# zyc-123/InstanceDiff

Measured on AMD Instinct MI355X. Metric: denoising steps/sec (256x256 bs16), higher is better.
Workload: dtype f32; 1 GPU; 256x256 1-ch synthetic, 1000-step reverse chain, batch 16 per GPU, 2 UNet fwd + reverse update per step; global_batch=16, parallelism=replicas x1 (no collective)

## Files before the change

### instancediff_amd/csrc/conv_wino4.hip

```cpp
#include "conv_args.h"
#include "wino_common.h"

using idiff_detail::ConvArgs;

namespace {

using namespace idiff_wino;

constexpr int CK = 4;
constexpr int TW = 32, TH = 16;
constexpr int RCOLS = TW + 2;
constexpr int RS = 40;
constexpr int TRH = TH + 2;
constexpr int PS = TRH * RS;
constexpr int PSP = 768;
constexpr int NT = 512;
constexpr int NL = 6;
constexpr int R_FLOATS = NL * NT;
constexpr int V_FLOATS = 9 * 2 * 64 * 4;
constexpr int U_FLOATS = 9 * 4 * 64 * 4;

typedef float floatx2 __attribute__((ext_vector_type(2)));

struct Geo4 {
    int np;
    int total;
    int tiles_y8;
};

#ifdef IDIFF_WINO_SLOTS
#define SLOT_INIT long long sl_acc[10] = {0, 0, 0, 0, 0, 0, 0, 0, 0, 0}, sl_t = 0;
#define SLOT_START sl_t = __builtin_readcyclecounter();
#define SLOT_MARK(k)                                        \
    {                                                       \
        const long long t_ = __builtin_readcyclecounter();  \
        sl_acc[k] += t_ - sl_t;                             \
        sl_t = t_;                                          \
    }
#define SLOT_FINI                                                                                                                   \
    if (lane == 0) {                                                                                                                \
        long long w_ = 0;                                                                                                           \
        for (int q_ = 0; q_ < 9; ++q_) w_ += sl_acc[q_];                                                                            \
        atomicAdd((unsigned long long*)trace + 8 + 2 * wave, (unsigned long long)w_);                                               \
        atomicAdd((unsigned long long*)trace + 9 + 2 * wave, (unsigned long long)sl_acc[9]);                                        \
    }
#else
#define SLOT_INIT
#define SLOT_START
#define SLOT_MARK(k)
#define SLOT_FINI
#endif

template <int MODE, int SPEC, bool RAG, bool HEAVY, bool G16>
__device__ __forceinline__ void conv_wino4_body(const ConvArgs& a, const Geo4& g, float* smem TRACE_PARAM) {
    static_assert(!G16 || (MODE == IDIFF_CONV_NORMAL && SPEC != 2), "the 16-byte gather: contiguous pieces, LDS-DMA only");
    constexpr int HU = G16 ? 5 : 4, HR = 3;
    constexpr int N_U = HEAVY ? HU : 9 - HU;
    constexpr int NR = G16 ? (HEAVY ? HR : 3 - HR) : NL;
    float* const Rb = smem;
    float* const Vb = smem + 3 * R_FLOATS;
    float* const Ub = Vb + 2 * V_FLOATS;
    float* const econst = Ub + 2 * U_FLOATS;
    int* const gtab = reinterpret_cast<int*>(econst + 512);
    constexpr unsigned R_BYTES = R_FLOATS * 4, U_BYTES = U_FLOATS * 4;
    const unsigned lds_base = __builtin_amdgcn_readfirstlane((unsigned)reinterpret_cast<unsigned long long>(smem));
    const unsigned U_LDS0 = lds_base + (3 * R_FLOATS + 2 * V_FLOATS) * 4;

    const int tid = threadIdx.x;
    const int lane = tid & 63;
    const int wave = __builtin_amdgcn_readfirstlane(tid >> 6);
    const int k4 = lane >> 4;
    const int cb = wave & 3;
    const int tblk = wave >> 2;
    const int g16_u0 = HEAVY ? wave : 4 * HU + wave - 4, g16_r0 = HEAVY ? wave : 4 * HR + wave - 4;
    const int HWin = a.Hin * a.Win;
    const int nchunks = a.Cin / CK;

    constexpr int RSRC_FLAGS = 0x00020000;
    struct View {
        int b, co0, y0, x0;
    };
    const float *p0A = a.src0, *p1A = a.src0, *puA = a.wwino4, *p0B = a.src0, *p1B = a.src0, *puB = a.wwino4;
    View vA = {0, 0, 0, 0}, vB = {0, 0, 0, 0};
    int nrB = 0;
    unsigned omaskA = 0, omaskB = 0;
    int it_b = 0, it_cob = 0, it_px = 0, it_py = 0;
    const int tiles_y = g.np / a.tiles_x;
    int d_cob, d_px, d_py, d_b;
    {
        const int G0 = gridDim.x;
        d_cob = G0 % a.ncob;
        const int r1 = G0 / a.ncob;
        d_px = r1 % a.tiles_x;
        const int r2 = r1 / a.tiles_x;
        d_py = r2 % tiles_y;
        d_b = r2 / tiles_y;
    }
    auto decode_first = [&](int item) {
        it_cob = item % a.ncob;
        const int r1 = item / a.ncob;
        it_px = r1 % a.tiles_x;
        const int r2 = r1 / a.tiles_x;
        it_py = r2 % tiles_y;
        it_b = r2 / tiles_y;
    };
    auto advance_item = [&]() {
        it_cob += d_cob;
        int carry = it_cob >= a.ncob;
        it_cob -= carry ? a.ncob : 0;
        it_px += d_px + carry;
        carry = it_px >= a.tiles_x;
        it_px -= carry ? a.tiles_x : 0;
        it_py += d_py + carry;
        carry = it_py >= tiles_y;
        it_py -= carry ? tiles_y : 0;
        it_b += d_b + carry;
    };
    auto decode_B = [&]() {
        vB.b = it_b, vB.co0 = it_cob * 64, vB.y0 = it_py * TH, vB.x0 = it_px * TW;
        puB = scalar_ptr(a.wwino4 + (long long)it_cob * U_FLOATS);
        p0B = scalar_ptr(a.src0 + (long long)it_b * a.bs0);
        p1B = scalar_ptr(SPEC == 3 ? a.src1 + (long long)it_b * a.bs1 : a.src0);
        nrB = 0x7fffffff;
    };
    auto write_table = [&](const View& v) {
        unsigned om;
        if (G16) gather_decode16<NT, NR, 256, PSP / 4, PS / 4, RS / 4>(tid, g16_r0 * 64 + lane, om, v.y0, v.x0, a, gtab, HWin);
        else gather_decode<MODE, NT, NL, PSP, PS, RS, RCOLS>(tid, om, v.y0, v.x0, a, gtab, HWin);
        return om;
    };
    auto shift_B_to_A = [&]() { p0A = p0B, p1A = p1B, puA = puB, vA = vB, omaskA = omaskB; };
    const int ustride_b = a.ncob * U_FLOATS * 4;

    typedef const __attribute__((address_space(4))) floatx4* cfloatx4p;
    struct Pro {
        floatx4 a, b;
    };
    auto load_pro = [&](int p) {
        Pro r;
        if (SPEC == 2) {
            const bool inA = p < nchunks;
            const long long o = (long long)(inA ? vA.b : vB.b) * a.C0r + (inA ? p : p - nchunks) * CK;
            r.a = *(cfloatx4p)(a.pro_a + o);
            r.b = *(cfloatx4p)(a.pro_b + o);
        }
        return r;
    };

    const unsigned u_voff = tid * 16;
    const unsigned l_voff = lane * 16;
    auto dma_u_piece16 = [&](int p, int buf, int i) {
        const bool inA = p < nchunks;
        const unsigned ub = (unsigned)(g16_u0 + 4 * i) * 1024u;
        const int so = (inA ? p : p - nchunks) * ustride_b + (int)ub;
        const __amdgpu_buffer_rsrc_t rsu = __builtin_amdgcn_make_buffer_rsrc(const_cast<float*>(inA ? puA : puB), 0, inA ? 0x7fffffff : nrB, RSRC_FLAGS);
        const unsigned lds0 = __builtin_amdgcn_readfirstlane(U_LDS0 + (unsigned)buf * U_BYTES + ub);
        asm volatile("s_nop 4\n\ts_mov_b32 m0, %2\n\ts_nop 0\n\tbuffer_load_dwordx4 %0, %1, %3 offen lds" ::"v"(l_voff), "s"(rsu), "s"(lds0), "s"(so) : "memory");
    };
    auto dma_u = [&](int p, int buf) {
        if (G16) {
#pragma unroll
            for (int i = 0; i < N_U; ++i) dma_u_piece16(p, buf, i);
            return;
        }
        const bool inA = p < nchunks;
        const int so = (inA ? p : p - nchunks) * ustride_b;
        const __amdgpu_buffer_rsrc_t rsu = __builtin_amdgcn_make_buffer_rsrc(const_cast<float*>(inA ? puA : puB), 0, inA ? 0x7fffffff : nrB, RSRC_FLAGS);
        const unsigned lds0 = __builtin_amdgcn_readfirstlane(U_LDS0 + (unsigned)buf * U_BYTES + (unsigned)wave * 1024u);
        asm volatile(
            "s_nop 4\n\ts_mov_b32 m0, %2\n\ts_nop 0\n\tbuffer_load_dwordx4 %0, %1, %3 offen lds\n\t"
            "s_add_u32 m0, m0, 0x2000\n\ts_nop 0\n\tbuffer_load_dwordx4 %0, %1, %4 offen lds\n\t"
            "s_add_u32 m0, m0, 0x2000\n\ts_nop 0\n\tbuffer_load_dwordx4 %0, %1, %5 offen lds\n\t"
            "s_add_u32 m0, m0, 0x2000\n\ts_nop 0\n\tbuffer_load_dwordx4 %0, %1, %6 offen lds"
            ::"v"(u_voff), "s"(rsu), "s"(lds0), "s"(so), "s"(so + NT * 16), "s"(so + 2 * NT * 16), "s"(so + 3 * NT * 16)
            : "memory", "scc");
        if (!HEAVY) {
            const unsigned lds4 = __builtin_amdgcn_readfirstlane(lds0 + 4 * NT * 16 - 256 * 16);
            asm volatile("s_nop 4\n\ts_mov_b32 m0, %2\n\ts_nop 0\n\tbuffer_load_dwordx4 %0, %1, %3 offen lds" ::"v"(u_voff), "s"(rsu), "s"(lds4),
                         "s"(so + 4 * NT * 16 - 256 * 16)
                         : "memory");
        }
    };
    auto dma_u_piece = [&](int p, int buf, int i) {
        if (G16) return dma_u_piece16(p, buf, i);
        const bool inA = p < nchunks;
        const int so = (inA ? p : p - nchunks) * ustride_b + (i < 4 ? i * NT * 16 : 4 * NT * 16 - 256 * 16);
        const __amdgpu_buffer_rsrc_t rsu = __builtin_amdgcn_make_buffer_rsrc(const_cast<float*>(inA ? puA : puB), 0, inA ? 0x7fffffff : nrB, RSRC_FLAGS);
        const unsigned lds0 = __builtin_amdgcn_readfirstlane(U_LDS0 + (unsigned)buf * U_BYTES + (unsigned)wave * 1024u + (unsigned)(i < 4 ? i * NT * 16 : 4 * NT * 16 - 256 * 16));
        asm volatile("s_nop 4\n\ts_mov_b32 m0, %2\n\ts_nop 0\n\tbuffer_load_dwordx4 %0, %1, %3 offen lds" ::"v"(u_voff), "s"(rsu), "s"(lds0), "s"(so) : "memory");
    };
    auto dma_raw = [&](int p, unsigned rslot) {
        const bool inA = p < nchunks;
        const int cbase = (inA ? p : p - nchunks) * CK;
        int goff[NL];
#pragma unroll
        for (int i = 0; i < NL; ++i) goff[i] = gtab[i * NT + tid];
        const int C0v = a.C0v;
        const bool second = SPEC == 3 && cbase >= C0v;
        const unsigned long long b0 = reinterpret_cast<unsigned long long>(inA ? p0A : p0B), b1 = reinterpret_cast<unsigned long long>(inA ? p1A : p1B);
        const float* const base = reinterpret_cast<const float*>(second ? b1 : b0);
        const int so = (second ? cbase - C0v : cbase) * HWin * 4;
        const __amdgpu_buffer_rsrc_t rs = __builtin_amdgcn_make_buffer_rsrc(const_cast<float*>(base), 0, inA ? 0x7fffffff : nrB, RSRC_FLAGS);
        const unsigned lds0 = __builtin_amdgcn_readfirstlane(lds_base + rslot + (unsigned)wave * 256u);
        asm volatile(
            "s_nop 4\n\ts_mov_b32 m0, %8\n\ts_nop 0\n\tbuffer_load_dword %0, %6, %7 offen lds\n\t"
            "s_add_u32 m0, m0, 0x800\n\ts_nop 0\n\tbuffer_load_dword %1, %6, %7 offen lds\n\t"
            "s_add_u32 m0, m0, 0x800\n\ts_nop 0\n\tbuffer_load_dword %2, %6, %7 offen lds\n\t"
            "s_add_u32 m0, m0, 0x800\n\ts_nop 0\n\tbuffer_load_dword %3, %6, %7 offen lds\n\t"
            "s_add_u32 m0, m0, 0x800\n\ts_nop 0\n\tbuffer_load_dword %4, %6, %7 offen lds\n\t"
            "s_add_u32 m0, m0, 0x800\n\ts_nop 0\n\tbuffer_load_dword %5, %6, %7 offen lds"
            ::"v"(goff[0]), "v"(goff[1]), "v"(goff[2]), "v"(goff[3]), "v"(goff[4]), "v"(goff[5]), "s"(rs), "s"(so), "s"(lds0)
            : "memory", "scc");
    };
    auto dma_raw_piece = [&](int p, unsigned rslot, int i, int goff_i) {
        const bool inA = p < nchunks;
        const int cbase = (inA ? p : p - nchunks) * CK;
        const int C0v = a.C0v;
        const bool second = SPEC == 3 && cbase >= C0v;
        const unsigned long long b0 = reinterpret_cast<unsigned long long>(inA ? p0A : p0B), b1 = reinterpret_cast<unsigned long long>(inA ? p1A : p1B);
        const float* const base = reinterpret_cast<const float*>(second ? b1 : b0);
        const int so = (second ? cbase - C0v : cbase) * HWin * 4;
        const __amdgpu_buffer_rsrc_t rs = __builtin_amdgcn_make_buffer_rsrc(const_cast<float*>(base), 0, inA ? 0x7fffffff : nrB, RSRC_FLAGS);
        if (G16) {
            const unsigned lds16 = __builtin_amdgcn_readfirstlane(lds_base + rslot + (unsigned)(g16_r0 + 4 * i) * 1024u);
            asm volatile("s_nop 4\n\ts_mov_b32 m0, %3\n\ts_nop 0\n\tbuffer_load_dwordx4 %0, %1, %2 offen lds" ::"v"(goff_i), "s"(rs), "s"(so), "s"(lds16) : "memory");
            return;
        }
        const unsigned lds0 = __builtin_amdgcn_readfirstlane(lds_base + rslot + (unsigned)wave * 256u + (unsigned)i * 2048u);
        asm volatile("s_nop 4\n\ts_mov_b32 m0, %3\n\ts_nop 0\n\tbuffer_load_dword %0, %1, %2 offen lds" ::"v"(goff_i), "s"(rs), "s"(so), "s"(lds0) : "memory");
    };
    auto dma_raw_fill = [&](int p, unsigned rslot) {
        if (G16) {
#pragma unroll
            for (int i = 0; i < NR; ++i) dma_raw_piece(p, rslot, i, gtab[i * NT + tid]);
        } else {
            dma_raw(p, rslot);
        }
    };
    float rinA[NL], rinB[NL];
    auto ld_raw = [&](float (&dst)[NL], int p, int i, int goff_i) {
        const bool inA = p < nchunks;
        const int so = (inA ? p : p - nchunks) * CK * HWin * 4;
        const __amdgpu_buffer_rsrc_t rs = __builtin_amdgcn_make_buffer_rsrc(const_cast<float*>(inA ? p0A : p0B), 0, inA ? 0x7fffffff : nrB, RSRC_FLAGS);
        asm volatile("s_nop 4\n\tbuffer_load_dword %0, %1, %2, %3 offen" : "=v"(dst[i]) : "v"(goff_i), "s"(rs), "s"(so) : "memory");
    };
    auto stage_act = [&](const float (&src)[NL], int p, const Pro& pro, unsigned rslot, int i0, int i1) {
        const unsigned om = p < nchunks ? omaskA : omaskB;
        float* const R = reinterpret_cast<float*>(reinterpret_cast<char*>(Rb) + rslot) + tid;
        constexpr bool hiw = !HEAVY;
#pragma unroll
        for (int i = 0; i < NL; ++i) {
            if (i < i0 || i >= i1) continue;
            const float pa = i == 0 ? pro.a.x : i == 1 ? (hiw ? pro.a.y : pro.a.x) : i == 2 ? pro.a.y : i == 3 ? pro.a.z : i == 4 ? (hiw ? pro.a.w : pro.a.z) : pro.a.w;
            const float pb = i == 0 ? pro.b.x : i == 1 ? (hiw ? pro.b.y : pro.b.x) : i == 2 ? pro.b.y : i == 3 ? pro.b.z : i == 4 ? (hiw ? pro.b.w : pro.b.z) : pro.b.w;
            const float x = silu_fast(pa * src[i] + pb);
            R[i * NT] = ((om >> i) & 1u) ? 0.f : x;
        }
    };

    constexpr bool heavy = HEAVY;
    const int trole = wave & 1;
    const int thalf = (wave >> 1) & 1;
    const int tx = lane & 7, tyl = (lane >> 3) & 1;
    const float al = trole ? -1.f : -4.f, be = trole ? 2.f : 1.f;
    const float* const trbase = Rb + k4 * PSP + (4 * (2 * thalf + tyl) + (heavy ? 1 : trole)) * RS + 4 * tx;
    const int ufirst = heavy ? 1 + 2 * trole : 5 * trole;
    float* const vwbase = Vb + thalf * 256 + lane * 4;
    float ta[6], tb[6], tlo[6], thi[6];
    struct Row16 {
        floatx4 lo, mid, hi;
    };
    Row16 ra, rb;
    auto rd_row = [&](const float* p, float (&d)[6], Row16& w) {
        if (G16) {
            w.lo = *reinterpret_cast<const floatx4*>(p);
            w.mid = *reinterpret_cast<const floatx4*>(p + 4);
            w.hi = *reinterpret_cast<const floatx4*>(p + 8);
            return;
        }
        const floatx4 lo = *reinterpret_cast<const floatx4*>(p);
        const floatx2 hi = *reinterpret_cast<const floatx2*>(p + 4);
        d[0] = lo.x, d[1] = lo.y, d[2] = lo.z, d[3] = lo.w, d[4] = hi.x, d[5] = hi.y;
    };
    auto take_row = [&](float (&d)[6], Row16& w) {
        if (!G16) return;
        asm volatile("" : "+v"(w.lo), "+v"(w.hi));
        d[0] = w.lo.w, d[1] = w.mid.x, d[2] = w.mid.y, d[3] = w.mid.z, d[4] = w.mid.w, d[5] = w.hi.x;
    };
    auto tr_piece = [&](int piece, unsigned rslot, int buf) {
        const float* p = reinterpret_cast<const float*>(reinterpret_cast<const char*>(trbase) + rslot);
        if (piece == 0) {
            if (heavy) rd_row(p + 1 * RS, ta, ra), rd_row(p + 3 * RS, tb, rb);
            else rd_row(p, ta, ra), rd_row(p + 2 * RS, tb, rb);
        } else if (piece == 1) {
            take_row(ta, ra), take_row(tb, rb);
            if (heavy) {
#pragma unroll
                for (int c = 0; c < 6; ++c) tlo[c] = __builtin_fmaf(al, ta[c], tb[c]);
                rd_row(p, ta, ra), rd_row(p + 2 * RS, tb, rb);
            } else {
#pragma unroll
                for (int c = 0; c < 6; ++c) tlo[c] = __builtin_fmaf(4.f, ta[c], -5.f * tb[c]);
                rd_row(p + 4 * RS, ta, ra);
            }
        } else if (piece == 2) {
            take_row(ta, ra);
            if (heavy) take_row(tb, rb);
            if (heavy) {
#pragma unroll
                for (int c = 0; c < 6; ++c) {
                    const float X = tlo[c], Y = __builtin_fmaf(al, ta[c], tb[c]);
                    tlo[c] = __builtin_fmaf(be, Y, X);
                    thi[c] = __builtin_fmaf(-be, Y, X);
                }
            } else {
#pragma unroll
                for (int c = 0; c < 6; ++c) tlo[c] += ta[c];
            }
        } else {
            const int which = piece - 3;
            if (which == 1 && !heavy) return;
            float o[6];
            bt6(which ? thi : tlo, o);
            const int u = ufirst + which;
            float* const V = vwbase + buf * V_FLOATS;
            *reinterpret_cast<floatx4*>(V + PF(u) * 512) = floatx4{o[0], o[1], o[2], o[3]};
            *reinterpret_cast<floatx2*>(V + PH(u) * 512 + 2 * (u & 1)) = floatx2{o[4], o[5]};
        }
    };

    const int G = gridDim.x;
    const int first = (int)xcd_remap(blockIdx.x, G);
    const int last = g.total;
    if (first >= last) return;
    auto fetch_consts = [&](const View& v) {
        float e = 0.f;
        if (HEAVY) {
            const int which = tid >> 6, co = v.co0 + (tid & 63);
            if (co < a.Cout) {
                if (which == 0 && a.bias) e = a.bias[co];
                if (which == 1 && a.vec) e = a.vec[(long long)v.b * a.Cout + co];
                if (which == 2 && a.aux) e = a.aux_a[(long long)v.b * a.Cout + co];
                if (which == 3 && a.aux) e = a.aux_b[(long long)v.b * a.Cout + co];
            }
        }
        return e;
    };
    TRACE_INIT(8)
    SLOT_INIT

    decode_first(first);
    decode_B();
    shift_B_to_A();
    omaskA = write_table(vA);
    if (first + G < last) {
        advance_item();
        decode_B();
    } else {
        nrB = 0, vB = vA;
    }
    {
        const float e0 = fetch_consts(vA);
        if (HEAVY) econst[tid] = e0;
    }
    dma_u(0, 0);
    if (SPEC != 2) {
        dma_raw_fill(0, 0 * R_BYTES);
        dma_raw_fill(1, 1 * R_BYTES);
        dma_raw_fill(2, 2 * R_BYTES);
        asm volatile("s_waitcnt vmcnt(%0)" ::"n"(NR) : "memory");
        __syncthreads();
    } else {
        int goff[NL];
#pragma unroll
        for (int i = 0; i < NL; ++i) goff[i] = gtab[i * NT + tid];
#pragma unroll
        for (int i = 0; i < NL; ++i) ld_raw(rinA, 0, i, goff[i]);
#pragma unroll
        for (int i = 0; i < NL; ++i) ld_raw(rinB, 1, i, goff[i]);
        const Pro pro0 = load_pro(0), pro1 = load_pro(1);
        asm volatile("s_waitcnt vmcnt(0)" : "+v"(rinA[0]), "+v"(rinA[1]), "+v"(rinA[2]), "+v"(rinA[3]), "+v"(rinA[4]), "+v"(rinA[5]), "+v"(rinB[0]),
                     "+v"(rinB[1]), "+v"(rinB[2]), "+v"(rinB[3]), "+v"(rinB[4]), "+v"(rinB[5])::"memory");
        stage_act(rinA, 0, pro0, 0 * R_BYTES, 0, NL);
        stage_act(rinB, 1, pro1, 1 * R_BYTES, 0, NL);
#pragma unroll
        for (int i = 0; i < NL; ++i) ld_raw(rinA, 2, i, goff[i]);
        __syncthreads();
    }
#pragma unroll
    for (int piece = 0; piece < 5; ++piece) tr_piece(piece, 0 * R_BYTES, 0);
    if (SPEC == 2) asm volatile("s_waitcnt vmcnt(0)" : "+v"(rinA[0]), "+v"(rinA[1]), "+v"(rinA[2]), "+v"(rinA[3]), "+v"(rinA[4]), "+v"(rinA[5])::"memory");
    else asm volatile("s_waitcnt vmcnt(0)" ::: "memory");
    __syncthreads();
    dma_u(1, 1);

    unsigned r_t = 1 * R_BYTES, r_a = 2 * R_BYTES, r_x = 0 * R_BYTES;
    int epar = 0;
    bool young = false;
    for (int item = first; item < last; item += G) {
        TRACE_MARK(0)
        TRACE_LAP(3)
        floatx4 acc[36];
        {
            const int opoff = lane * 4;
            floatx4 ob[2], oa[2];
            ob[0] = *reinterpret_cast<const floatx4*>(Vb + tblk * 256 + opoff);
            oa[0] = *reinterpret_cast<const floatx4*>(Ub + cb * 256 + opoff);
            auto chunk = [&](int cc, auto par_tag, auto zero_tag) {
                constexpr int PAR = decltype(par_tag)::value;
                constexpr bool ZERO = decltype(zero_tag)::value;
                const float* V = Vb + PAR * V_FLOATS + tblk * 256 + opoff;
                const float* U = Ub + PAR * U_FLOATS + cb * 256 + opoff;
                const float* Vn = Vb + (PAR ^ 1) * V_FLOATS + tblk * 256 + opoff;
                const float* Un = Ub + (PAR ^ 1) * U_FLOATS + cb * 256 + opoff;
                int goff[NL];
                if (cc + 3 == nchunks) omaskB = write_table(vB);
#pragma unroll
                for (int i = 0; i < NL; ++i) goff[i] = i < NR ? gtab[i * NT + tid] : 0;
                float(&rin_s)[NL] = PAR ? rinB : rinA;
                float(&rin_l)[NL] = PAR ? rinA : rinB;
                Pro pro;
                if (SPEC == 2) pro = load_pro(cc + 2);
                SLOT_START
#pragma unroll
                for (int q = 0; q < 9; ++q) {
                    if (q + 1 < 9) {
                        ob[(q + 1 + PAR) & 1] = *reinterpret_cast<const floatx4*>(V + (q + 1) * 512);
                        oa[(q + 1 + PAR) & 1] = *reinterpret_cast<const floatx4*>(U + (q + 1) * 1024);
                    } else {
                        if (young) asm volatile("s_waitcnt vmcnt(%0)" ::"n"(NR + (RAG ? 0 : 16)) : "memory");
                        else asm volatile("s_waitcnt vmcnt(%0)" ::"n"(NR) : "memory");
                        young = false;
                        __builtin_amdgcn_sched_barrier(0);
                        SLOT_MARK(8)
                        __syncthreads();
                        SLOT_MARK(9)
                        if (cc + 1 == nchunks) dma_u(cc + 2, PAR);
                        else dma_u_piece(cc + 2, PAR, 0);
                        ob[PAR ^ 1] = *reinterpret_cast<const floatx4*>(Vn);
                        oa[PAR ^ 1] = *reinterpret_cast<const floatx4*>(Un);
                    }
                    const floatx4 bv = ob[(q + PAR) & 1], av = oa[(q + PAR) & 1];
                    const floatx4 z4 = floatx4{0.f, 0.f, 0.f, 0.f};
                    acc[4 * q + 0] = __builtin_amdgcn_mfma_f32_16x16x4f32(av.x, bv.x, ZERO ? z4 : acc[4 * q + 0], 0, 0, 0);
                    acc[4 * q + 1] = __builtin_amdgcn_mfma_f32_16x16x4f32(av.y, bv.y, ZERO ? z4 : acc[4 * q + 1], 0, 0, 0);
                    acc[4 * q + 2] = __builtin_amdgcn_mfma_f32_16x16x4f32(av.z, bv.z, ZERO ? z4 : acc[4 * q + 2], 0, 0, 0);
                    acc[4 * q + 3] = __builtin_amdgcn_mfma_f32_16x16x4f32(av.w, bv.w, ZERO ? z4 : acc[4 * q + 3], 0, 0, 0);
                    if (!ZERO) {
                        if (!G16) {
                            if (q < 3) dma_u_piece(cc + 1, PAR ^ 1, q + 1);
                            if (q == 3 && !HEAVY) dma_u_piece(cc + 1, PAR ^ 1, 4);
                        }
                    }
                    if (SPEC == 2 && q == 5) {
                        if (young) asm volatile("s_waitcnt vmcnt(%6)" : "+v"(rin_s[0]), "+v"(rin_s[1]), "+v"(rin_s[2]), "+v"(rin_s[3]), "+v"(rin_s[4]), "+v"(rin_s[5]) : "n"(N_U + 2 + (RAG ? 0 : 16)) : "memory");
                        else asm volatile("s_waitcnt vmcnt(%6)" : "+v"(rin_s[0]), "+v"(rin_s[1]), "+v"(rin_s[2]), "+v"(rin_s[3]), "+v"(rin_s[4]), "+v"(rin_s[5]) : "n"(N_U + 2) : "memory");
                        stage_act(rin_s, cc + 2, pro, r_a, 0, 2);
                    }
                    if (SPEC == 2 && q == 6) stage_act(rin_s, cc + 2, pro, r_a, 2, 4);
                    if (SPEC == 2 && q == 7) stage_act(rin_s, cc + 2, pro, r_a, 4, 6);
                    auto req = [&](int i) {
                        if (SPEC == 2) ld_raw(rin_l, cc + 3, i, goff[i]);
                        else dma_raw_piece(cc + 3, r_x, i, goff[i]);
                    };
                    if (G16) {
                        static_assert(!G16 || N_U - 1 + NR <= 8, "a piece at quad 8 would lie behind the counted wait");
                        if (q < N_U - 1) {
                            if (!ZERO) dma_u_piece(cc + 1, PAR ^ 1, q + 1);
                        } else if (q < N_U - 1 + NR) {
                            req(q - (N_U - 1));
                        }
                    } else {
                        if (HEAVY && q == 3) req(0);
                        if (!HEAVY && q == 4) req(0);
                        if (q == 4) req(1);
                        if (q == 5) req(2);
                        if (q == 6) req(3);
                        if (q == 7) req(4), req(5);
                    }
                    if (q < 5) tr_piece(q, r_t, PAR ^ 1);
                    __builtin_amdgcn_sched_barrier(0);
                    if (q < 8) { SLOT_MARK(q) }
                }
                const unsigned t = r_t;
                r_t = r_a, r_a = r_x, r_x = t;
            };
            chunk(0, std::integral_constant<int, 0>{}, std::true_type{});
            chunk(1, std::integral_constant<int, 1>{}, std::false_type{});
            for (int cc = 2; cc < nchunks; cc += 2) {
                chunk(cc, std::integral_constant<int, 0>{}, std::false_type{});
                chunk(cc + 1, std::integral_constant<int, 1>{}, std::false_type{});
            }
        }
        TRACE_MARK(1)

        const View v = vA;
        const float* const ebase_item = econst + epar * 256;
        const bool more = item + G < last;
        float pre_e = 0.f;
        if (more) {
            shift_B_to_A();
            if (item + 2 * G < last) {
                advance_item();
                decode_B();
            } else {
                nrB = 0, vB = vA;
            }
            pre_e = fetch_consts(vA);
        }
        young = true;

        const int b = v.b, co0 = v.co0, y0 = v.y0, x0 = v.x0;
        {
            int lane_e = lane;
            asm volatile("" : "+v"(lane_e));
            const int j = lane_e & 15, k4 = lane_e >> 4;
            const int HWo = a.Hout * a.Wout;
            const int ty0 = y0 + 8 * tblk;
            const bool wave_live = co0 + cb * 16 < a.Cout;
            const long long wave_org = (long long)(co0 + cb * 16) * HWo + (long long)ty0 * a.Wout + x0;
            const __amdgpu_buffer_rsrc_t rso = __builtin_amdgcn_make_buffer_rsrc(const_cast<float*>(scalar_ptr(a.out + (long long)b * a.obs + wave_org)), 0, wave_live ? 0x7fffffff : 0, RSRC_FLAGS);
            const float* const resb = a.res ? a.res + (long long)b * a.rbs + wave_org : nullptr;
            const float* const auxb = a.aux ? a.aux + (long long)b * a.abs_ + wave_org : nullptr;
            const bool inside = !RAG || ((ty0 + 4 * (j >> 3) < a.Hout) && (x0 + 4 * (j & 7) < a.Wout));
            const unsigned lane_off = (unsigned)(4 * k4) * (unsigned)HWo + (unsigned)(4 * (j >> 3)) * (unsigned)a.Wout + 4u * (j & 7);
            const float* const ebase = ebase_item + cb * 16 + 4 * k4;
            const bool want_stats = a.stats != nullptr && ty0 < a.Hout && wave_live;
            const bool has_res = a.res != nullptr && wave_live, has_aux = a.aux != nullptr && wave_live;
            const float* const stbase = a.stats ? a.stats + (((long long)b * a.ntiles + (ty0 >> 3) * a.tiles_x + (x0 >> 5)) * a.Cout + co0 + cb * 16) * 2 : a.out;
            const __amdgpu_buffer_rsrc_t rst = __builtin_amdgcn_make_buffer_rsrc(const_cast<float*>(scalar_ptr(stbase)), 0, want_stats ? 0x7fffffff : 0, RSRC_FLAGS);
            constexpr int AUX_SC1 = 1 << 4;
            float zz[6][4][4];
#pragma unroll
            for (int u = 0; u < 6; ++u) {
#pragma unroll
                for (int r = 0; r < 4; ++r) {
                    at6(acc[pos(u, 0)][r], acc[pos(u, 1)][r], acc[pos(u, 2)][r], acc[pos(u, 3)][r], acc[pos(u, 4)][r], acc[pos(u, 5)][r], zz[u][r]);
                    asm volatile("" : "+v"(zz[u][r][0]), "+v"(zz[u][r][1]), "+v"(zz[u][r][2]), "+v"(zz[u][r][3]));
                }
                __builtin_amdgcn_sched_barrier(0);
            }
            TRACE_MARK(2)
            floatx4 nres = floatx4{0.f, 0.f, 0.f, 0.f}, naux = nres;
#ifdef W4_STATS_LAST
            typedef unsigned uintx2_ __attribute__((ext_vector_type(2)));
            uintx2_ spr[4];
#endif
            auto fetch = [&](int s) {
                if (!inside) return;
                const long long so = (long long)(s >> 2) * HWo + (s & 3) * a.Wout;
                if (has_res) nres = *reinterpret_cast<const floatx4*>(resb + so + lane_off);
                if (has_aux) naux = *reinterpret_cast<const floatx4*>(auxb + so + lane_off);
            };
            fetch(0);
#pragma unroll
            for (int r = 0; r < 4; ++r) {
                const float bv = ebase[r];
                float y[4][4];
#pragma unroll
                for (int x = 0; x < 4; ++x) {
                    float col[4];
                    at6(zz[0][r][x], zz[1][r][x], zz[2][r][x], zz[3][r][x], zz[4][r][x], zz[5][r][x], col);
#pragma unroll
                    for (int dy = 0; dy < 4; ++dy) y[dy][x] = col[dy] + bv;
                }
                {
                    float ssum = 0.f, ssq = 0.f;
                    if (a.stats != nullptr) {
#pragma unroll
                        for (int dy = 0; dy < 4; ++dy) {
                            ssum += (y[dy][0] + y[dy][1]) + (y[dy][2] + y[dy][3]);
                            ssq += (y[dy][0] * y[dy][0] + y[dy][1] * y[dy][1]) + (y[dy][2] * y[dy][2] + y[dy][3] * y[dy][3]);
                        }
                        if (!inside) ssum = 0.f, ssq = 0.f;
                        ssum = row_sum16(ssum);
                        ssq = row_sum16(ssq);
                    }
                    typedef unsigned uintx2 __attribute__((ext_vector_type(2)));
                    const uintx2 pr = {__builtin_bit_cast(unsigned, ssum), __builtin_bit_cast(unsigned, ssq)};
#ifndef W4_STATS_LAST
                    __builtin_amdgcn_raw_buffer_store_b64(pr, rst, j == 15 ? (4 * k4 + r) * 8 : -1, 0, AUX_SC1);
#else
                    spr[r] = pr;
#endif
                }
                const float add = ebase[64 + r];
                float aa = 0.f, ab = 0.f;
                if (has_aux) aa = ebase[128 + r], ab = ebase[192 + r];
#pragma unroll
                for (int dy = 0; dy < 4; ++dy) {
                    const floatx4 cres = nres, caux = naux;
                    if (4 * r + dy + 1 < 16) fetch(4 * r + dy + 1);
                    floatx4 v4 = floatx4{y[dy][0] + add, y[dy][1] + add, y[dy][2] + add, y[dy][3] + add};
                    if (has_res) v4 += cres;
                    if (has_aux) {
                        v4.x += silu_fast(aa * caux.x + ab), v4.y += silu_fast(aa * caux.y + ab);
                        v4.z += silu_fast(aa * caux.z + ab), v4.w += silu_fast(aa * caux.w + ab);
                    }
                    typedef unsigned uintx4 __attribute__((ext_vector_type(4)));
                    if (!RAG || inside) __builtin_amdgcn_raw_buffer_store_b128(__builtin_bit_cast(uintx4, v4), rso, (int)(lane_off * 4u), (r * HWo + dy * a.Wout) * 4, 0);
                }
                __builtin_amdgcn_sched_barrier(0);
            }
#ifdef W4_STATS_LAST
#pragma unroll
            for (int r = 0; r < 4; ++r) __builtin_amdgcn_raw_buffer_store_b64(spr[r], rst, j == 15 ? (4 * k4 + r) * 8 : -1, 0, AUX_SC1);
#endif
        }
        TRACE_MARK(3)
        if (HEAVY && more) econst[(epar ^ 1) * 256 + tid] = pre_e;
        epar ^= 1;
    }
    asm volatile("s_waitcnt vmcnt(0)" ::: "memory");
    TRACE_FINI(8)
    SLOT_FINI
}

template <int MODE, int SPEC, bool RAG>
__global__ __launch_bounds__(NT) void conv_wino4_kernel(const ConvArgs a, const Geo4 g TRACE_PARAM) {
    extern __shared__ __attribute__((aligned(16))) float smem[];
#ifdef IDIFF_WINO_TRACE
    if (__builtin_amdgcn_readfirstlane(threadIdx.x >> 6) < 4) conv_wino4_body<MODE, SPEC, RAG, true, false>(a, g, smem, trace);
    else conv_wino4_body<MODE, SPEC, RAG, false, false>(a, g, smem, trace);
#else
    if (__builtin_amdgcn_readfirstlane(threadIdx.x >> 6) < 4) conv_wino4_body<MODE, SPEC, RAG, true, false>(a, g, smem);
    else conv_wino4_body<MODE, SPEC, RAG, false, false>(a, g, smem);
#endif
}

template <int SPEC, bool RAG>
__global__ __launch_bounds__(NT) void conv_wino4_g16_kernel(const ConvArgs a, const Geo4 g TRACE_PARAM) {
    extern __shared__ __attribute__((aligned(16))) float smem[];
#ifdef IDIFF_WINO_TRACE
    if (__builtin_amdgcn_readfirstlane(threadIdx.x >> 6) < 4) conv_wino4_body<IDIFF_CONV_NORMAL, SPEC, RAG, true, true>(a, g, smem, trace);
    else conv_wino4_body<IDIFF_CONV_NORMAL, SPEC, RAG, false, true>(a, g, smem, trace);
#else
    if (__builtin_amdgcn_readfirstlane(threadIdx.x >> 6) < 4) conv_wino4_body<IDIFF_CONV_NORMAL, SPEC, RAG, true, true>(a, g, smem);
    else conv_wino4_body<IDIFF_CONV_NORMAL, SPEC, RAG, false, true>(a, g, smem);
#endif
}

template <auto KERN>
int launch_items(const ConvArgs& a, hipStream_t st) {
    const size_t lds = ((size_t)3 * R_FLOATS + 2 * V_FLOATS + 2 * U_FLOATS + 2 * 256 + NL * NT) * sizeof(float);
    static idiff_dyn_lds_cache lds_cache;
    auto kern = KERN;
    if (const int rc = idiff_dyn_lds(lds_cache, kern, lds, "conv2d(winograd4)")) return rc;
    int num_cu = 0;
    if (!idiff_num_cu(&num_cu)) IDIFF_FAIL(IDIFF_E_HIP, "conv2d(winograd4): cannot query the CU count");
    Geo4 g;
    const int tiles_y16 = (a.Hout + TH - 1) / TH;
    g.np = a.tiles_x * tiles_y16;
    g.tiles_y8 = (a.Hout + 7) / 8;
    const long long total = (long long)a.B * g.np * a.ncob;
    if (total >= (1ll << 31)) IDIFF_FAIL(IDIFF_E_BADARG, "conv2d(winograd4): grid too large");
    g.total = (int)total;
    int per = 0;
    const int grid = persistent_grid(g.total, num_cu, &per);
#ifdef IDIFF_WINO_TRACE
    static long long* tr = nullptr;
    if (!tr) (void)hipMalloc(&tr, 32 * sizeof(long long));
    (void)hipMemsetAsync(tr, 0, 32 * sizeof(long long), st);
    hipLaunchKernelGGL(kern, dim3(grid), dim3(NT), lds, st, a, g, tr);
    long long h[32];
    (void)hipMemcpyAsync(h, tr, sizeof(h), hipMemcpyDeviceToHost, st);
    (void)hipStreamSynchronize(st);
    fprintf(stderr, "[wino4 trace] Cin=%d Cout=%d H=%d items=%d per=%d | main loop %lld | switch + output transform %lld | statistics + stores %lld | to next item %lld (cycles/item, wave 0)\n",
            a.Cin, a.Cout, a.Hout, g.total, per, h[0] / g.total, h[1] / g.total, h[2] / g.total, h[3] / g.total);
#ifdef IDIFF_WINO_SLOTS
    {
        const long long nch = (long long)g.total * (a.Cin / CK - 1);
        fprintf(stderr, "[wino4 slots] Cin=%d H=%d work/barrier-wait cycles per chunk, waves 0..7:", a.Cin, a.Hout);
        for (int w = 0; w < 8; ++w) fprintf(stderr, " %lld/%lld", h[8 + 2 * w] / nch, h[9 + 2 * w] / nch);
        fprintf(stderr, "\n");
    }
#endif
#else
    hipLaunchKernelGGL(kern, dim3(grid), dim3(NT), lds, st, a, g);
#endif
    IDIFF_CHECK_LAUNCH("conv2d_fwd(winograd4)");
    return IDIFF_OK;
}

template <int MODE, int SPEC, bool RAG>
int launch_rag(const ConvArgs& a, hipStream_t st) {
    if constexpr (MODE == IDIFF_CONV_NORMAL && SPEC != 2) {
        const bool al0 = !(reinterpret_cast<uintptr_t>(a.src0) & 15) && !(a.bs0 & 3) && !(a.Win & 3);
        const bool al1 = SPEC != 3 || (!(reinterpret_cast<uintptr_t>(a.src1) & 15) && !(a.bs1 & 3));
        if (al0 && al1) return launch_items<conv_wino4_g16_kernel<SPEC, RAG>>(a, st);
    }
    return launch_items<conv_wino4_kernel<MODE, SPEC, RAG>>(a, st);
}

__global__ void pack_wino4_kernel(const float* __restrict__ w, float* __restrict__ out, int Cout, int Cin, int transpose) {
    const int Co = transpose ? Cin : Cout, Ci = transpose ? Cout : Cin;
    const int ncob = (Co + 63) / 64;
    const long long n = (long long)Co * Ci;
    for (long long i = blockIdx.x * (long long)blockDim.x + threadIdx.x; i < n; i += (long long)gridDim.x * blockDim.x) {
        const int co = i % Co, ci = i / Co;
        float gk[3][3];
        load_taps(w, Cin, co, ci, transpose, gk);
        float t[6][3];
#pragma unroll
        for (int q = 0; q < 3; ++q) {
            float o[6];
            g6(gk[0][q], gk[1][q], gk[2][q], o);
#pragma unroll
            for (int u = 0; u < 6; ++u) t[u][q] = o[u];
        }
        const int cc = ci >> 2, kk = ci & 3;
        const int cbk = co >> 6, col = co & 63, cb = col >> 4, i16 = col & 15;
        float* dst = out + ((long long)cc * ncob + cbk) * U_FLOATS + cb * 256 + (kk * 16 + i16) * 4;
#pragma unroll
        for (int u = 0; u < 6; ++u) {
            float o[6];
            g6(t[u][0], t[u][1], t[u][2], o);
#pragma unroll
            for (int v = 0; v < 6; ++v) {
                const int p = pos(u, v);
                dst[(p >> 2) * 1024 + (p & 3)] = o[v];
            }
        }
    }
}

int wino4_mode() {
    static const int m = [] {
        const char* e = getenv("IDIFF_WINOGRAD4");
        return e ? atoi(e) : 1;
    }();
    return m;
}
}

namespace idiff_detail {

long long conv_wino4_items(const ConvArgs& a, int ks, int mode, bool requested) {
    if (ks != 3 || !a.wwino4 || (wino4_mode() == 0 && !requested)) return 0;
    if (mode != IDIFF_CONV_NORMAL && mode != IDIFF_CONV_UPSAMPLE2) return 0;
    if (a.Cout % 16 || a.Cin % 8 || a.C0v % CK || (a.Hout & 3) || (a.Wout & 3) || a.Wout < 24) return 0;
    if ((long long)a.Cin * a.Hin * a.Win * 4 >= (1ll << 31)) return 0;
    if (144ll * a.Cin * a.ncob * 64 + U_FLOATS * 4 >= (1ll << 31)) return 0;
    if (mode == IDIFF_CONV_UPSAMPLE2 && (a.pro_a || a.src1)) return 0;
    if (a.pro_a && a.src1) return 0;
    if (a.pro_a && ((a.C0r & 3) || (reinterpret_cast<uintptr_t>(a.pro_a) & 15) || (reinterpret_cast<uintptr_t>(a.pro_b) & 15))) return 0;
    if ((reinterpret_cast<uintptr_t>(a.wwino4) & 15) != 0) return 0;
    if ((a.obs & 3) || (a.res && (a.rbs & 3)) || (a.aux && (a.abs_ & 3))) return 0;
    if ((reinterpret_cast<uintptr_t>(a.out) & 15) || (reinterpret_cast<uintptr_t>(a.res) & 15) || (reinterpret_cast<uintptr_t>(a.aux) & 15)) return 0;
    return (long long)a.tiles_x * ((a.Hout + TH - 1) / TH) * a.ncob;
}

int launch_conv_wino4(const ConvArgs& a, int mode, hipStream_t st) {
#ifdef W4_ONLY
    return launch_rag<IDIFF_CONV_NORMAL, 1, false>(a, st);
#else
    return launch_spec_ladder(mode, a.pro_a != nullptr, a.src1 != nullptr, a.Hout % TH || a.Wout % TW, [&](auto mode_tag, auto spec_tag, auto rag_tag) {
        return launch_rag<decltype(mode_tag)::value, decltype(spec_tag)::value, decltype(rag_tag)::value>(a, st);
    });
#endif
}

}

extern "C" int idiff_pack_conv_weight_wino4(const float* w, float* wwino4, int Cout, int Cin, int transpose, idiff_stream_t stream) {
    return pack_entry<36>("pack_conv_weight_wino4", pack_wino4_kernel, w, wwino4, Cout, Cin, transpose, stream);
}
```

### instancediff_amd/csrc/wino_common.h

```cpp
#pragma once
#include <stdlib.h>

#include <type_traits>

#include "common.h"

namespace idiff_detail {
bool winograd_disabled();
}

namespace idiff_wino {


template <int CTRL>
__device__ __forceinline__ float dpp_row_shr(float v) {
    return __builtin_bit_cast(float, __builtin_amdgcn_update_dpp(0, __builtin_bit_cast(int, v), CTRL, 0xf, 0xf, true));
}
__device__ __forceinline__ float row_sum16(float v) {
    v += dpp_row_shr<0x111>(v);
    v += dpp_row_shr<0x112>(v);
    v += dpp_row_shr<0x114>(v);
    v += dpp_row_shr<0x118>(v);
    return v;
}

template <typename T>
__device__ __forceinline__ T* scalar_ptr(const T* p) {
    const unsigned long long v = reinterpret_cast<unsigned long long>(p);
    const unsigned lo = __builtin_amdgcn_readfirstlane((unsigned)v), hi = __builtin_amdgcn_readfirstlane((unsigned)(v >> 32));
    return reinterpret_cast<T*>(((unsigned long long)hi << 32) | lo);
}


__host__ __device__ constexpr int PF(int u) { return (3 * u + 1) / 2; }
__host__ __device__ constexpr int PH(int u) { return 1 + 3 * (u / 2); }
__host__ __device__ constexpr int pos(int u, int v) { return v < 4 ? 4 * PF(u) + v : 4 * PH(u) + 2 * (u & 1) + (v - 4); }

__device__ __forceinline__ void bt6(const float (&x)[6], float (&o)[6]) {
    o[0] = __builtin_fmaf(4.f, x[0], __builtin_fmaf(-5.f, x[2], x[4]));
    const float p = __builtin_fmaf(-4.f, x[2], x[4]), q = __builtin_fmaf(-4.f, x[1], x[3]);
    o[1] = p + q;
    o[2] = p - q;
    const float c = x[4] - x[2], e = x[3] - x[1];
    o[3] = __builtin_fmaf(2.f, e, c);
    o[4] = __builtin_fmaf(-2.f, e, c);
    o[5] = __builtin_fmaf(4.f, x[1], __builtin_fmaf(-5.f, x[3], x[5]));
}
__device__ __forceinline__ void at6(const float x0, const float x1, const float x2, const float x3, const float x4, const float x5, float (&o)[4]) {
    const float s1 = x1 + x2, d1 = x1 - x2, s2 = x3 + x4, d2 = x3 - x4;
    o[0] = (x0 + s1) + s2;
    o[1] = __builtin_fmaf(2.f, d2, d1);
    o[2] = __builtin_fmaf(4.f, s2, s1);
    o[3] = __builtin_fmaf(8.f, d2, d1) + x5;
}
__device__ __forceinline__ void a6(float x0, float x1, float x2, float x3, float (&o)[6]) {
    const float s = x0 + x2, t = x1 + x3;
    o[0] = x0;
    o[1] = s + t;
    o[2] = s - t;
    const float p = __builtin_fmaf(4.f, x2, x0), q = __builtin_fmaf(8.f, x3, 2.f * x1);
    o[3] = p + q;
    o[4] = p - q;
    o[5] = x3;
}
__device__ __forceinline__ void g6(float x0, float x1, float x2, float (&o)[6]) {
    o[0] = 0.25f * x0;
    const float s = x0 + x2;
    o[1] = (-1.f / 6.f) * (s + x1);
    o[2] = (-1.f / 6.f) * (s - x1);
    const float t = __builtin_fmaf(4.f, x2, x0);
    o[3] = (1.f / 24.f) * __builtin_fmaf(2.f, x1, t);
    o[4] = (1.f / 24.f) * __builtin_fmaf(-2.f, x1, t);
    o[5] = x2;
}
__device__ __forceinline__ void gt3(float m0, float m1, float m2, float m3, float m4, float m5, float (&o)[3]) {
    const float s12 = m1 + m2, d12 = m1 - m2, s34 = m3 + m4, d34 = m3 - m4;
    o[0] = __builtin_fmaf(0.25f, m0, __builtin_fmaf(-1.f / 6.f, s12, (1.f / 24.f) * s34));
    o[1] = __builtin_fmaf(-1.f / 6.f, d12, (1.f / 12.f) * d34);
    o[2] = __builtin_fmaf(-1.f / 6.f, s12, __builtin_fmaf(1.f / 6.f, s34, m5));
}

template <int MODE, int NT, int NL, int PSP, int PS, int RS, int RCOLS, typename Args>
__device__ __forceinline__ void gather_decode(const int& tid, unsigned& om, const int& y0, const int& x0, const Args& a, int* const& gtab, const int& HWin) {
    int t = tid;
    asm volatile("" : "+v"(t));
    om = 0;
#pragma unroll
    for (int i = 0; i < NL; ++i) {
        const int e = t + i * NT;
        const int ci = e / PSP;
        const int rem = e - ci * PSP;
        const int r = rem / RS;
        const int c = rem - r * RS;
        const int oy = y0 - 1 + r, ox = x0 - 1 + c;
        const bool in = rem < PS && c < RCOLS && (unsigned)oy < (unsigned)a.Hout && (unsigned)ox < (unsigned)a.Wout;
        const int sp = MODE == IDIFF_CONV_UPSAMPLE2 ? (oy >> 1) * a.Win + (ox >> 1) : oy * a.Win + ox;
        gtab[i * NT + tid] = in ? (ci * HWin + sp) * 4 : -1;
        om |= (in ? 0u : 1u) << i;
    }
}

template <int NT, int NR, int ES, int PSP4, int PS4, int RS4, typename Args>
__device__ __forceinline__ void gather_decode16(const int& tid, const int& e0, unsigned& om, const int& y0, const int& x0, const Args& a, int* const& gtab, const int& HWin) {
    int t = e0;
    asm volatile("" : "+v"(t));
    om = 0;
#pragma unroll
    for (int i = 0; i < NR; ++i) {
        const int e = t + i * ES;
        const int ci = e / PSP4;
        const int rem = e - ci * PSP4;
        const int r = rem / RS4;
        const int j = rem - r * RS4;
        const int oy = y0 - 1 + r, ox4 = x0 - 4 + 4 * j;
        const bool in = rem < PS4 && (unsigned)oy < (unsigned)a.Hout && (unsigned)ox4 < (unsigned)a.Wout;
        gtab[i * NT + tid] = in ? (ci * HWin + oy * a.Win + ox4) * 4 : -1;
        om |= (in ? 0u : 1u) << i;
    }
}

__device__ __forceinline__ void load_taps(const float* __restrict__ w, int Cin, int co, int ci, int transpose, float (&g)[3][3]) {
#pragma unroll
    for (int p = 0; p < 3; ++p)
#pragma unroll
        for (int q = 0; q < 3; ++q)
            g[p][q] = transpose ? w[((long long)ci * Cin + co) * 9 + (2 - p) * 3 + (2 - q)] : w[((long long)co * Cin + ci) * 9 + p * 3 + q];
}


template <int NPOS, typename K>
int pack_entry(const char* name, K kern, const float* w, float* image, int Cout, int Cin, int transpose, idiff_stream_t stream) {
    IDIFF_CHECK_ARG(w && image && Cout > 0 && Cin > 0, "%s: bad args", name);
    const int Co = transpose ? Cin : Cout, Ci = transpose ? Cout : Cin;
    IDIFF_CHECK_ARG(Co % 16 == 0 && Ci % 8 == 0, "%s: needs conv Cout %% 16 == 0 and Cin %% 8 == 0 (got %d, %d)", name, Co, Ci);
    if (Co % 64) {
        hipError_t e = hipMemsetAsync(image, 0, (size_t)NPOS * Ci * ((Co + 63) / 64) * 64 * sizeof(float), (hipStream_t)stream);
        if (e != hipSuccess) IDIFF_FAIL(IDIFF_E_HIP, "%s: hipMemsetAsync: %s", name, hipGetErrorString(e));
    }
    const long long n = (long long)Cout * Cin;
    const int grid = (int)((n + 255) / 256 > 4096 ? 4096 : (n + 255) / 256);
    hipLaunchKernelGGL(kern, dim3(grid), dim3(256), 0, (hipStream_t)stream, w, image, Cout, Cin, transpose);
    IDIFF_CHECK_LAUNCH(name);
    return IDIFF_OK;
}

inline int persistent_grid(int total, int slots, int* per_out = nullptr) {
    const int per = (total + slots - 1) / slots;
    if (per_out) *per_out = per;
    return (total + per - 1) / per;
}

template <typename F>
int launch_spec_ladder(int mode, bool pro, bool src1, bool ragged, F&& launch) {
    auto rag = [&](auto mode_tag, auto spec_tag) {
        if (ragged) return launch(mode_tag, spec_tag, std::true_type{});
        return launch(mode_tag, spec_tag, std::false_type{});
    };
    using Normal = std::integral_constant<int, IDIFF_CONV_NORMAL>;
    using Upsample = std::integral_constant<int, IDIFF_CONV_UPSAMPLE2>;
    if (mode == IDIFF_CONV_UPSAMPLE2) return rag(Upsample{}, std::integral_constant<int, 1>{});
    if (pro) return rag(Normal{}, std::integral_constant<int, 2>{});
    if (src1) return rag(Normal{}, std::integral_constant<int, 3>{});
    return rag(Normal{}, std::integral_constant<int, 1>{});
}

}

#ifdef IDIFF_WINO_TRACE
#define TRACE_PARAM , long long* trace
#define TRACE_INIT(N) long long tr_t[(N) + 1] = {0}, tr_acc[N] = {0};
#define TRACE_MARK(k)                       \
    tr_t[k] = __builtin_readcyclecounter(); \
    if (k > 0) tr_acc[k - 1] += tr_t[k] - tr_t[k - 1];
#define TRACE_LAP(last) \
    if (tr_t[last] != 0) tr_acc[last] += tr_t[0] - tr_t[last];
#define TRACE_FINI(N)                                                                                                   \
    if (tid == 0) {                                                                                                     \
        for (int q_ = 0; q_ < (N); ++q_) atomicAdd((unsigned long long*)trace + q_, (unsigned long long)tr_acc[q_]);    \
    }
#else
#define TRACE_PARAM
#define TRACE_INIT(N)
#define TRACE_MARK(k)
#define TRACE_LAP(last)
#define TRACE_FINI(N)
#endif
```

Baseline: 44.45 steps/s.

## Skip dead Winograd positions in upsample-mode F(4,3) conv

For the 2x-upsample conv mode, Winograd domain row and column 2 are treated as dead, because the nearest-upsampled input's structure is taken to make them contribute nothing. The change drops the MFMAs, operand LDS loads, input-transform work and output-transform terms for those positions. It uses compile-time live masks per quad and remaps the double-buffer parity across skipped quads. This cuts about 11 of 36 tensor-core products per channel chunk in upsample convs, at the cost of more complex buffer indexing. Correctness rests on the dead-position reasoning and the modified bt6 holding exactly.

New measurement: 44.94 steps/s, median of 6. 1.01x the previous value.

```diff
diff --git a/instancediff_amd/csrc/conv_wino4.hip b/instancediff_amd/csrc/conv_wino4.hip
--- a/instancediff_amd/csrc/conv_wino4.hip
+++ b/instancediff_amd/csrc/conv_wino4.hip
@@ -22,6 +22,19 @@
 
 typedef float floatx2 __attribute__((ext_vector_type(2)));
 
+template <bool UPSAMPLED>
+constexpr unsigned long long chunk_live() {
+    unsigned long long m = 0;
+    for (int q = 0; q < 9; ++q) m |= (unsigned long long)quad_live<UPSAMPLED>(q) << (4 * q);
+    return m;
+}
+template <bool UPSAMPLED>
+constexpr unsigned chunk_sets() {
+    unsigned m = 0, n = 0;
+    for (int q = 0; q < 9; ++q) m |= (n & 1u) << q, n += quad_live<UPSAMPLED>(q) != 0;
+    return m | (n & 1u) << 9;
+}
+
 struct Geo4 {
     int np;
     int total;
@@ -57,6 +70,7 @@
     constexpr int HU = G16 ? 5 : 4, HR = 3;
     constexpr int N_U = HEAVY ? HU : 9 - HU;
     constexpr int NR = G16 ? (HEAVY ? HR : 3 - HR) : NL;
+    constexpr bool UPS = MODE == IDIFF_CONV_UPSAMPLE2;
     float* const Rb = smem;
     float* const Vb = smem + 3 * R_FLOATS;
     float* const Ub = Vb + 2 * V_FLOATS;
@@ -307,11 +321,16 @@
             take_row(ta, ra);
             if (heavy) take_row(tb, rb);
             if (heavy) {
-#pragma unroll
-                for (int c = 0; c < 6; ++c) {
-                    const float X = tlo[c], Y = __builtin_fmaf(al, ta[c], tb[c]);
-                    tlo[c] = __builtin_fmaf(be, Y, X);
-                    thi[c] = __builtin_fmaf(-be, Y, X);
+                if (UPS && !trole) {
+#pragma unroll
+                    for (int c = 0; c < 6; ++c) tlo[c] = __builtin_fmaf(be, __builtin_fmaf(al, ta[c], tb[c]), tlo[c]);
+                } else {
+#pragma unroll
+                    for (int c = 0; c < 6; ++c) {
+                        const float X = tlo[c], Y = __builtin_fmaf(al, ta[c], tb[c]);
+                        tlo[c] = __builtin_fmaf(be, Y, X);
+                        thi[c] = __builtin_fmaf(-be, Y, X);
+                    }
                 }
             } else {
 #pragma unroll
@@ -320,8 +339,9 @@
         } else {
             const int which = piece - 3;
             if (which == 1 && !heavy) return;
+            if (UPS && which == 1 && !trole) return;
             float o[6];
-            bt6(which ? thi : tlo, o);
+            bt6<UPS>(which ? thi : tlo, o);
             const int u = ufirst + which;
             float* const V = vwbase + buf * V_FLOATS;
             *reinterpret_cast<floatx4*>(V + PF(u) * 512) = floatx4{o[0], o[1], o[2], o[3]};
@@ -411,6 +431,11 @@
                 constexpr bool ZERO = decltype(zero_tag)::value;
                 const float* V = Vb + PAR * V_FLOATS + tblk * 256 + opoff;
                 const float* U = Ub + PAR * U_FLOATS + cb * 256 + opoff;
+                constexpr unsigned long long LIVE = chunk_live<UPS>();
+                constexpr unsigned SETS = chunk_sets<UPS>();
+                static_assert((LIVE >> 32) != 0 && (LIVE & 0xf) != 0, "quads 0 and 8 carry the chunk's first and last operand requests");
+                auto qlive = [](int q) { return (unsigned)(LIVE >> (4 * q)) & 0xfu; };
+                auto qset = [](int q, int par) { return (int)(((SETS >> q) ^ ((SETS >> 9) & (unsigned)par)) & 1u); };
                 const float* Vn = Vb + (PAR ^ 1) * V_FLOATS + tblk * 256 + opoff;
                 const float* Un = Ub + (PAR ^ 1) * U_FLOATS + cb * 256 + opoff;
                 int goff[NL];
@@ -424,9 +449,13 @@
                 SLOT_START
 #pragma unroll
                 for (int q = 0; q < 9; ++q) {
+                    const unsigned lm = qlive(q);
                     if (q + 1 < 9) {
-                        ob[(q + 1 + PAR) & 1] = *reinterpret_cast<const floatx4*>(V + (q + 1) * 512);
-                        oa[(q + 1 + PAR) & 1] = *reinterpret_cast<const floatx4*>(U + (q + 1) * 1024);
+                        if (lm) {
+                            const int nq = qlive(q + 1) ? q + 1 : q + 2;
+                            ob[qset(nq, PAR)] = *reinterpret_cast<const floatx4*>(V + nq * 512);
+                            oa[qset(nq, PAR)] = *reinterpret_cast<const floatx4*>(U + nq * 1024);
+                        }
                     } else {
                         if (young) asm volatile("s_waitcnt vmcnt(%0)" ::"n"(NR + (RAG ? 0 : 16)) : "memory");
                         else asm volatile("s_waitcnt vmcnt(%0)" ::"n"(NR) : "memory");
@@ -437,15 +466,17 @@
                         SLOT_MARK(9)
                         if (cc + 1 == nchunks) dma_u(cc + 2, PAR);
                         else dma_u_piece(cc + 2, PAR, 0);
-                        ob[PAR ^ 1] = *reinterpret_cast<const floatx4*>(Vn);
-                        oa[PAR ^ 1] = *reinterpret_cast<const floatx4*>(Un);
+                        ob[qset(0, PAR ^ 1)] = *reinterpret_cast<const floatx4*>(Vn);
+                        oa[qset(0, PAR ^ 1)] = *reinterpret_cast<const floatx4*>(Un);
                     }
-                    const floatx4 bv = ob[(q + PAR) & 1], av = oa[(q + PAR) & 1];
-                    const floatx4 z4 = floatx4{0.f, 0.f, 0.f, 0.f};
-                    acc[4 * q + 0] = __builtin_amdgcn_mfma_f32_16x16x4f32(av.x, bv.x, ZERO ? z4 : acc[4 * q + 0], 0, 0, 0);
-                    acc[4 * q + 1] = __builtin_amdgcn_mfma_f32_16x16x4f32(av.y, bv.y, ZERO ? z4 : acc[4 * q + 1], 0, 0, 0);
-                    acc[4 * q + 2] = __builtin_amdgcn_mfma_f32_16x16x4f32(av.z, bv.z, ZERO ? z4 : acc[4 * q + 2], 0, 0, 0);
-                    acc[4 * q + 3] = __builtin_amdgcn_mfma_f32_16x16x4f32(av.w, bv.w, ZERO ? z4 : acc[4 * q + 3], 0, 0, 0);
+                    if (lm) {
+                        const floatx4 bv = ob[qset(q, PAR)], av = oa[qset(q, PAR)];
+                        const floatx4 z4 = floatx4{0.f, 0.f, 0.f, 0.f};
+                        if (lm & 1u) acc[4 * q + 0] = __builtin_amdgcn_mfma_f32_16x16x4f32(av.x, bv.x, ZERO ? z4 : acc[4 * q + 0], 0, 0, 0);
+                        if (lm & 2u) acc[4 * q + 1] = __builtin_amdgcn_mfma_f32_16x16x4f32(av.y, bv.y, ZERO ? z4 : acc[4 * q + 1], 0, 0, 0);
+                        if (lm & 4u) acc[4 * q + 2] = __builtin_amdgcn_mfma_f32_16x16x4f32(av.z, bv.z, ZERO ? z4 : acc[4 * q + 2], 0, 0, 0);
+                        if (lm & 8u) acc[4 * q + 3] = __builtin_amdgcn_mfma_f32_16x16x4f32(av.w, bv.w, ZERO ? z4 : acc[4 * q + 3], 0, 0, 0);
+                    }
                     if (!ZERO) {
                         if (!G16) {
                             if (q < 3) dma_u_piece(cc + 1, PAR ^ 1, q + 1);
@@ -531,11 +562,13 @@
             const __amdgpu_buffer_rsrc_t rst = __builtin_amdgcn_make_buffer_rsrc(const_cast<float*>(scalar_ptr(stbase)), 0, want_stats ? 0x7fffffff : 0, RSRC_FLAGS);
             constexpr int AUX_SC1 = 1 << 4;
             float zz[6][4][4];
+            auto m = [&](int u, int v, int r) { return pos_live<UPS>(u, v) ? acc[pos(u, v)][r] : 0.f; };
 #pragma unroll
             for (int u = 0; u < 6; ++u) {
+                if (UPS && u == 2) continue;
 #pragma unroll
                 for (int r = 0; r < 4; ++r) {
-                    at6(acc[pos(u, 0)][r], acc[pos(u, 1)][r], acc[pos(u, 2)][r], acc[pos(u, 3)][r], acc[pos(u, 4)][r], acc[pos(u, 5)][r], zz[u][r]);
+                    at6(m(u, 0, r), m(u, 1, r), m(u, 2, r), m(u, 3, r), m(u, 4, r), m(u, 5, r), zz[u][r]);
                     asm volatile("" : "+v"(zz[u][r][0]), "+v"(zz[u][r][1]), "+v"(zz[u][r][2]), "+v"(zz[u][r][3]));
                 }
                 __builtin_amdgcn_sched_barrier(0);
@@ -560,7 +593,7 @@
 #pragma unroll
                 for (int x = 0; x < 4; ++x) {
                     float col[4];
-                    at6(zz[0][r][x], zz[1][r][x], zz[2][r][x], zz[3][r][x], zz[4][r][x], zz[5][r][x], col);
+                    at6(zz[0][r][x], zz[1][r][x], UPS ? 0.f : zz[2][r][x], zz[3][r][x], zz[4][r][x], zz[5][r][x], col);
 #pragma unroll
                     for (int dy = 0; dy < 4; ++dy) y[dy][x] = col[dy] + bv;
                 }
diff --git a/instancediff_amd/csrc/wino_common.h b/instancediff_amd/csrc/wino_common.h
--- a/instancediff_amd/csrc/wino_common.h
+++ b/instancediff_amd/csrc/wino_common.h
@@ -36,11 +36,25 @@
 __host__ __device__ constexpr int PH(int u) { return 1 + 3 * (u / 2); }
 __host__ __device__ constexpr int pos(int u, int v) { return v < 4 ? 4 * PF(u) + v : 4 * PH(u) + 2 * (u & 1) + (v - 4); }
 
+template <bool UPSAMPLED>
+__host__ __device__ constexpr bool pos_live(int u, int v) {
+    return !UPSAMPLED || (u != 2 && v != 2);
+}
+template <bool UPSAMPLED>
+__host__ __device__ constexpr unsigned quad_live(int quad) {
+    unsigned m = 0;
+    for (int u = 0; u < 6; ++u)
+        for (int v = 0; v < 6; ++v)
+            if (pos_live<UPSAMPLED>(u, v) && pos(u, v) / 4 == quad) m |= 1u << (pos(u, v) & 3);
+    return m;
+}
+
+template <bool UPSAMPLED = false>
 __device__ __forceinline__ void bt6(const float (&x)[6], float (&o)[6]) {
     o[0] = __builtin_fmaf(4.f, x[0], __builtin_fmaf(-5.f, x[2], x[4]));
     const float p = __builtin_fmaf(-4.f, x[2], x[4]), q = __builtin_fmaf(-4.f, x[1], x[3]);
     o[1] = p + q;
-    o[2] = p - q;
+    o[2] = UPSAMPLED ? p : p - q;
     const float c = x[4] - x[2], e = x[3] - x[1];
     o[3] = __builtin_fmaf(2.f, e, c);
     o[4] = __builtin_fmaf(-2.f, e, c);
```
